# yhlleo/DWC-GAN

Hardware: AMD Instinct MI355X
Metric: CelebA 128x128 training images/sec (higher is better)
Workload: dtype f32; 1 GPU; BASELINE configs[1]: CelebA-shaped 128x128, per-GPU batch 16, fp32, full iteration (dis_update + gen_update + EMA + LR step), vgg_w=0, stride-1 3x3 / 5x5 and stride-2 4x4 layers (forward, data and weight gradient) as fp32-accurate TWO-plane f16 split products on the f16 MFMA (hi + lo 2^-11 per operand, per-tensor power-of-two scales, 3 products per multiply-add, matrix-core partial sums flushed to; image_size=128, per_gpu_batch=16, global_batch=16, parallelism=dp1

## Files before the change

dwc-gan_amd/csrc/conv_fold.h:

```cpp
#pragma once
#include "conv_geom.h"

namespace {

__device__ __forceinline__ int reflect_src(int p, int n, int pad, int (&out)[3]) {
    int c = 0;
    out[c++] = p + pad;
    if (p >= 1 && p <= pad) out[c++] = pad - p;
    if (p >= n - 1 - pad && p <= n - 2) out[c++] = pad + 2 * (n - 1) - p;
    return c;
}

template <typename T>
__global__ void fold_reflect_kernel(const T* __restrict__ gp, T* __restrict__ dx, int B, int H, int W, int C4, int pad,
                                    int Wp) {
    const size_t idx = (size_t)blockIdx.x * blockDim.x + threadIdx.x;
    const size_t total = (size_t)B * H * W * C4;
    if (idx >= total) return;
    const int c = idx % C4;
    size_t r = idx / C4;
    const int w = r % W;
    r /= W;
    const int h = r % H;
    const int n = r / H;
// ... 126 lines not shown
            else e = off_right / 4 + ((size_t)(n * H + rh - pad) * pad + rw - pad - W) * C4;
            for (int p = 0; p < parts; ++p) s += ld4(ring + p * part_stride, e + c);
        }
    st4(dx, o, s);
}

template <typename T>
int fold_ring(T* dx, const float* ring, const SameDgrad& f, int B, int H, int W, int C, int pad, hipStream_t st) {
    const size_t total = (size_t)B * 2 * pad * (W + H) * (C / 4);
    hipLaunchKernelGGL(fold_ring_kernel<T>, dim3((unsigned)((total + 255) / 256)), dim3(256), 0, st, dx, ring, f.ring_elems[0],
                       f.ring_elems[0] + f.ring_elems[1], f.ring_elems[0] + f.ring_elems[1] + f.ring_elems[2], f.parts, f.ring_total,
                       B, H, W, C / 4, pad);
    DWC_LAUNCH_CHECK();
    return DWC_OK;
}

template <typename T>
__global__ __launch_bounds__(256) void splitk_reduce_kernel(const float* __restrict__ part, T* __restrict__ dst,
                                                            const float* __restrict__ bias, size_t total4, size_t stride4, int splits,
                                                            int N, int act) {
    const int nq = N >> 2;
    for (size_t i = (size_t)blockIdx.x * blockDim.x + threadIdx.x; i < total4; i += (size_t)gridDim.x * blockDim.x) {
        f32x4 s = ld4(part, i);
        for (int z = 1; z < splits; ++z) s += ld4(part, (size_t)z * stride4 + i);
        const int c4 = i % nq;
        if (bias) s += ld4(bias, c4);
#pragma unroll
        for (int k = 0; k < 4; ++k) s[k] = dwc_act_apply(s[k], act, c4 * 4 + k);
        st4(dst, i, s);
    }
}

template <typename T>
int splitk_reduce(const float* part, T* dst, const float* bias, size_t dst_elems, int splits, int N, int act, hipStream_t st) {
    const size_t total4 = dst_elems / 4;
    size_t blocks = (total4 + 255) / 256;
    if (blocks > 2048) blocks = 2048;
    hipLaunchKernelGGL(splitk_reduce_kernel<T>, dim3((unsigned)blocks), dim3(256), 0, st, part, dst, bias, total4, total4, splits, N, act);
    DWC_LAUNCH_CHECK();
    return DWC_OK;
}

template <typename T>
__global__ void weight_prepare_fwd_kernel(const float* __restrict__ w, T* __restrict__ out, int Cout, int Cin, int KHW,
                                          int cout_pad, int cin_pad, int Kp) {
    const size_t idx = (size_t)blockIdx.x * blockDim.x + threadIdx.x;
    if (idx >= (size_t)cout_pad * Kp) return;
    const int k = idx % Kp, co = idx / Kp;
    const int ci = k % cin_pad, tap = k / cin_pad;
    float v = 0.f;
    if (co < Cout && ci < Cin && tap < KHW) v = w[((size_t)co * Cin + ci) * KHW + tap];
    out[idx] = (T)v;
}

template <typename T>
__global__ void weight_prepare_dgrad_kernel(const float* __restrict__ w, T* __restrict__ out, int Cout, int Cin, int KH, int KW,
                                            int stride, int cout_pad, int cin_pad, int Kp) {
    const size_t idx = (size_t)blockIdx.x * blockDim.x + threadIdx.x;
    const size_t per_class = (size_t)cin_pad * Kp;
    const int classes = stride == 1 ? 1 : 4;
    if (idx >= per_class * classes) return;
// ... 49 lines not shown
```

dwc-gan_amd/csrc/conv_geom.h:

```cpp
#pragma once
#include <stdio.h>
#include <stdlib.h>
#include <string.h>

#include "dwc_common.h"

namespace {

struct Gather {
    const void* src;
    int SH, SW, SC, logSC;
    int OH, OW;
    int logOW, logOHW;
    int KH, KW, kw_magic;
    int mul_h, mul_w, kstep, off_h, off_w;
    int reflect;
    int M, K;
    int tap_t;
};

struct Scatter {
    void* dst;
    int N;
    int OHf, OWf, os;
// ... 10 lines not shown
    Gather g;
    Scatter o;
    const void* w;
    int kt0, kt1, tiles, tiles_n;
    int oph, opw;
};
struct StripSet {
    Strip s[8];
    int kt_per_part;
    size_t part_stride;
};

__global__ void wgrad_reduce_kernel(const float* __restrict__ slab, float* __restrict__ dw, int splits, int K, int N, int Cin,
                                    int KHW, int cin_real, int cout_real) {
    const size_t idx = (size_t)blockIdx.x * blockDim.x + threadIdx.x;
    if (idx >= (size_t)K * N) return;
    const int co = idx % N;
    const int k = idx / N;
    const int ci = k % Cin, tap = k / Cin;
    if (co >= cout_real || ci >= cin_real) return;
    float s = 0.f;
    for (int z = 0; z < splits; ++z) s += slab[(size_t)z * K * N + idx];
    dw[((size_t)co * cin_real + ci) * KHW + tap] = s;
}

__global__ __launch_bounds__(256) void wgrad_reduce_wide_kernel(const float* __restrict__ slab, float* __restrict__ dw, int splits, int K, int N,
                                                                int Cin, int KHW, int cin_real, int cout_real) {
    __shared__ float part[8][32];
    const int e = threadIdx.x & 31, g = threadIdx.x >> 5;
    const size_t total = (size_t)K * N;
    const size_t idx = (size_t)blockIdx.x * 32 + e;
    const int per = (splits + 7) / 8;
    const int z0 = g * per, z1 = min(splits, z0 + per);
    float s = 0.f;
    if (idx < total) {
        const float* p = slab + idx;
        int z = z0;
        for (; z + 8 <= z1; z += 8) {
            float v[8];
#pragma unroll
            for (int u = 0; u < 8; ++u) v[u] = p[(size_t)(z + u) * total];
#pragma unroll
            for (int u = 0; u < 8; ++u) s += v[u];
        }
        for (; z < z1; ++z) s += p[(size_t)z * total];
    }
// ... 3 lines not shown
#pragma unroll
    for (int q = 1; q < 8; ++q) s += part[q][e];
    const int co = idx % N;
    const int k = idx / N;
    const int ci = k % Cin, tap = k / Cin;
    if (co >= cout_real || ci >= cin_real) return;
    dw[((size_t)co * cin_real + ci) * KHW + tap] = s;
}

inline bool wgrad_reduce_takes_wide(int splits, int K, int N) { return splits >= 16 && (size_t)K * N <= 262144; }

inline bool wgrad_reduce_wide(const float* slab, float* dw, int splits, int K, int N, int Cin, int KHW, int cin_real, int cout_real,
                              hipStream_t st) {
    const size_t total = (size_t)K * N;
    if (!wgrad_reduce_takes_wide(splits, K, N)) return false;
    hipLaunchKernelGGL(wgrad_reduce_wide_kernel, dim3((unsigned)((total + 31) / 32)), dim3(256), 0, st, slab, dw, splits, K, N, Cin, KHW,
                       cin_real, cout_real);
    return true;
}

inline void wgrad_reduce(const float* slab, float* dw, int splits, int K, int N, int Cin, int KHW, int cin_real, int cout_real,
                         hipStream_t st) {
    if (wgrad_reduce_wide(slab, dw, splits, K, N, Cin, KHW, cin_real, cout_real, st)) return;
    const size_t total = (size_t)K * N;
    hipLaunchKernelGGL(wgrad_reduce_kernel, dim3((unsigned)((total + 255) / 256)), dim3(256), 0, st, slab, dw, splits, K, N, Cin, KHW,
                       cin_real, cout_real);
}

int kw_magic_for(int KW, int max_tap) {
    const int magic = (65536 + KW - 1) / KW;
    for (int tp = 0; tp <= max_tap; ++tp)
        if (((tp * magic) >> 16) != tp / KW) return -1;
    return magic;
}

constexpr int NUM_CU = 256;
struct Plan {
    int bm, bn, splits, kt_per_split;
};

struct TileCand { int bm, bn, resident; float f; };

template <size_t NC>
Plan plan_gemm(int M, int N, int K, int classes, int bk, const TileCand (&cands)[NC], int split_below) {
    const int nk = (K + bk - 1) / bk;
    Plan best = {128, 32, 1, nk};
    float best_cost = 3.0e38f;
    auto valid = [N](const TileCand& c) {
        if (N <= 32) return c.bn == 32;
// ... 312 lines not shown
```

dwc-gan_amd/csrc/conv_halo_bf16.hip:

```cpp
#include <type_traits>

#include "conv_geom.h"

namespace {

typedef __bf16 bf16;
typedef __bf16 bf16x8 __attribute__((ext_vector_type(8)));
typedef __bf16 bf16x4 __attribute__((ext_vector_type(4)));

constexpr int BK = 64;
constexpr int TB = 16;

__device__ __forceinline__ bf16x4 pack4h(float a, float b, float c, float d) {
    bf16x4 r;
    r[0] = (bf16)a; r[1] = (bf16)b; r[2] = (bf16)c; r[3] = (bf16)d;
    return r;
}

struct HaloArgs {
    const bf16* x;
    const bf16* w;
    const float* bias;
    const bf16* add;
    bf16* y;
// ... 460 lines not shown
    hipStream_t st = (hipStream_t)stream;
    const dim3 grid((Cin / (bn == 128 ? 64 : 128)) * a.n_tiles * a.tap_groups * splits);
#ifdef DWC_DEV_ABLATIONS
    static const int dbg = getenv("DWC_WGRAD_HALO_DBG") ? atoi(getenv("DWC_WGRAD_HALO_DBG")) : 0;
    if (K == 3 && dbg == 4) hipLaunchKernelGGL((wgrad_halo_kernel<3, 128, 4>), grid, dim3(512), 0, st, a);
    else
#endif
    const char* he = getenv("DWC_WGRAD_HALF");
    const int half = he ? atoi(he) : 1;
    if (zero) {
        if (K == 3) hipLaunchKernelGGL((wgrad_halo_kernel<3, 128, 0, 0, -1, 0, 0, true>), grid, dim3(512), 0, st, a);
        else if (K == 4) hipLaunchKernelGGL((wgrad_halo_kernel<4, 128, 0, 0, -1, 0, 0, true>), grid, dim3(512), 0, st, a);
        else if (bn == 128 && half) hipLaunchKernelGGL((wgrad_halo_kernel<5, 128, 0, 0, -1, 0, 1, true>), grid, dim3(512), 0, st, a);
        else if (bn == 128) hipLaunchKernelGGL((wgrad_halo_kernel<5, 128, 0, 0, -1, 0, 0, true>), grid, dim3(512), 0, st, a);
        else if (half) hipLaunchKernelGGL((wgrad_halo_kernel<5, 64, 0, 0, -1, 0, 1, true>), grid, dim3(512), 0, st, a);
        else hipLaunchKernelGGL((wgrad_halo_kernel<5, 64, 0, 0, -1, 0, 0, true>), grid, dim3(512), 0, st, a);
    } else if (K == 3) hipLaunchKernelGGL((wgrad_halo_kernel<3, 128>), grid, dim3(512), 0, st, a);
    else if (K == 4) hipLaunchKernelGGL((wgrad_halo_kernel<4, 128>), grid, dim3(512), 0, st, a);
    else if (bn == 128 && half) hipLaunchKernelGGL((wgrad_halo_kernel<5, 128, 0, 0, -1, 0, 1>), grid, dim3(512), 0, st, a);
    else if (bn == 128) hipLaunchKernelGGL((wgrad_halo_kernel<5, 128>), grid, dim3(512), 0, st, a);
    else if (half) hipLaunchKernelGGL((wgrad_halo_kernel<5, 64, 0, 0, -1, 0, 1>), grid, dim3(512), 0, st, a);
    else hipLaunchKernelGGL((wgrad_halo_kernel<5, 64>), grid, dim3(512), 0, st, a);
    DWC_LAUNCH_CHECK();
    const size_t total = (size_t)K * K * Cin * Cout;
    hipLaunchKernelGGL(wgrad_reduce_kernel, dim3((total + 255) / 256), dim3(256), 0, st, (const float*)ws, dw_oihw, splits,
                       K * K * Cin, Cout, Cin, K * K, cin_real, cout_real);
    DWC_LAUNCH_CHECK();
    return DWC_OK;
}

int dwc_bf16_conv2d_wgrad_halo(const void* x, const void* dy, float* dw_oihw, int B, int H, int W, int Cin, int Cout, int K,
                               int cin_real, int cout_real, void* ws, size_t ws_bytes, void* stream) {
    return wgrad_halo_run(x, dy, dw_oihw, B, H, W, Cin, Cout, K, cin_real, cout_real, ws, ws_bytes, stream, false);
}

int dwc_bf16_conv2d_wgrad_halo_zeropad(const void* x, const void* dy, float* dw_oihw, int B, int H, int W, int Cin, int Cout, int K,
                                       int cin_real, int cout_real, void* ws, size_t ws_bytes, void* stream) {
    if (!x || !dy || !dw_oihw) return DWC_EINVAL;
    return wgrad_halo_run(x, dy, dw_oihw, B, H, W, Cin, Cout, K, cin_real, cout_real, ws, ws_bytes, stream, true);
}

}
```

dwc-gan_amd/csrc/conv_halo_x3.hip:

```cpp
#include <type_traits>

#include "conv_geom.h"

namespace {

typedef __bf16 bf16;
typedef __bf16 bf16x8 __attribute__((ext_vector_type(8)));
typedef unsigned int u32x2 __attribute__((ext_vector_type(2)));

constexpr int TB = 16;
constexpr int CS = 16;

typedef float f32x2 __attribute__((ext_vector_type(2)));
__device__ __forceinline__ void split3(f32x4 v, u32x2& p0, u32x2& p1, u32x2& p2) {
#pragma unroll
    for (int k = 0; k < 2; ++k) {
        const f32x2 x = {v[2 * k], v[2 * k + 1]};
        const f32x2 hb = {__uint_as_float(__float_as_uint(x[0]) & 0xffff0000u), __uint_as_float(__float_as_uint(x[1]) & 0xffff0000u)};
        const f32x2 r = x - hb;
        const f32x2 mb = {__uint_as_float(__float_as_uint(r[0]) & 0xffff0000u), __uint_as_float(__float_as_uint(r[1]) & 0xffff0000u)};
        const f32x2 l = r - mb;
        p0[k] = __builtin_amdgcn_perm(__float_as_uint(x[1]), __float_as_uint(x[0]), 0x07060302u);
        p1[k] = __builtin_amdgcn_perm(__float_as_uint(r[1]), __float_as_uint(r[0]), 0x07060302u);
        p2[k] = __builtin_amdgcn_perm(__float_as_uint(l[1]), __float_as_uint(l[0]), 0x07060302u);
// ... 988 lines not shown
            }
            asm volatile("s_waitcnt lgkmcnt(0)" ::: "memory");
            __builtin_amdgcn_s_barrier();
            buf ^= 1;
            cur = nxt;
            nxt = unit_next(nxt);
        }
    }
    const int Ktot = KS * KS * a.Cin;
    float* out = a.slab + (size_t)(split * HALVES + half_id) * Ktot * a.N;
#pragma unroll
    for (int kh = 0; kh < KS; ++kh) {
        const int tap = kh * KS + kw;
#pragma unroll
        for (int r = 0; r < 16; ++r) {
            const int k = tap * a.Cin + cs * CIW + ci_tile * 32 + (r & 3) + 8 * (r >> 2) + 4 * hi;
            if constexpr (NPL == 2) out[(size_t)k * a.N + tn * BN + co_tile * 32 + l31] = acc[kh][r] * sx.inv * sdy.inv;
            else out[(size_t)k * a.N + tn * BN + co_tile * 32 + l31] = acc[kh][r] + lo[kh][r];
        }
    }
#endif
}

__global__ void x3_wgrad_reduce_kernel(const float* __restrict__ slab, float* __restrict__ dw, int splits, int K, int N, int Cin, int KHW,
                                       int cin_real, int cout_real) {
    const size_t idx = (size_t)blockIdx.x * blockDim.x + threadIdx.x;
    if (idx >= (size_t)K * N) return;
    const int co = idx % N;
    const int k = idx / N;
    const int ci = k % Cin, tap = k / Cin;
    if (co >= cout_real || ci >= cin_real) return;
    const float* p = slab + idx;
    const size_t stride = (size_t)K * N;
    float s = 0.f;
    int z = 0;
    for (; z + 4 <= splits; z += 4) {
        const float v0 = p[(size_t)z * stride], v1 = p[(size_t)(z + 1) * stride], v2 = p[(size_t)(z + 2) * stride],
                    v3 = p[(size_t)(z + 3) * stride];
        s += v0;
        s += v1;
        s += v2;
        s += v3;
    }
    for (; z < splits; ++z) s += p[(size_t)z * stride];
    dw[((size_t)co * cin_real + ci) * KHW + tap] = s;
}

static int x3_wgrad_ciw() { return 64; }

int x3_wgrad_bn(int B, int H, int W, int Cin, int Cout, int K) {
    if (K == 4) {
        if (B <= 0 || H < 8 || W < 32 || (H % 8) || (W % 32) || Cin < 64 || (Cin % 64)) return 0;
    } else if (B <= 0 || (K != 3 && K != 5) || H < 8 || W < 16 || (H % 8) || (W % 16) || Cin < 64 || (Cin % 64)) return 0;
    if ((size_t)B * H * W * Cin * 4 >= 0xffffffffull || (size_t)B * H * W * Cout * 4 >= 0xffffffffull) return 0;
    if (Cout >= 128 && !(Cout % 128)) return 128;
    return (Cout >= 64 && !(Cout % 64)) ? 64 : 0;
}

void x3_wgrad_plan(int B, int H, int W, int Cin, int Cout, int K, int bn, int npl, int* splits, int* ups) {
    const int ciw = x3_wgrad_ciw();
    const int roles = (Cin / ciw) * (Cout / bn) * K;
    const int units = K == 4 ? B * (H / 8) * (W / 32) : B * (H / 8) * (W / 16);
    const int cus = (npl == 2 && K != 5 && (long)units * roles >= 8L * 512) ? 512 : 256;
    const int smax = units / 4 > 0 ? units / 4 : 1;
    int s = 1;
    double best = 0.0;
    for (int c = 1; c <= smax && c * roles <= 2 * cus; ++c) {
        const int wgs = c * roles, rounds = (wgs + cus - 1) / cus;
        const double fill = (double)wgs / (rounds * cus) / (rounds > 1 ? 1.05 : 1.0);
// ... 337 lines not shown
    X3WgradArgs a;
    a.x = x; a.dy = dy; a.slab = (float*)ws;
    a.xs = (const unsigned long long*)xs; a.xs_epoch = xs_epoch; a.dys = (const unsigned long long*)dys; a.dys_epoch = dys_epoch;
    a.B = B; a.H = H; a.W = W; a.Cin = Cin; a.N = Cout;
    if (K == 4) {
        a.units_x = W / 32; a.units_per_img = (H / 8) * (W / 32);
    } else {
        a.units_x = W / 16; a.units_per_img = (H / 8) * (W / 16);
    }
    a.total_units = B * a.units_per_img; a.units_per_split = ups;
    a.n_tiles = Cout / bn;
    const int ciw = x3_wgrad_ciw();
    a.roles = (Cin / ciw) * a.n_tiles * K;
    hipStream_t st = (hipStream_t)stream;
    const dim3 grid(a.roles * splits);
    if (K == 4) {
        if (bn == 128) hipLaunchKernelGGL((wgrad_x3_kernel<4, 128, 64, 2, NPL, ZP>), grid, dim3(512), 0, st, a);
        else hipLaunchKernelGGL((wgrad_x3_kernel<4, 64, 64, 2, NPL, ZP>), grid, dim3(512), 0, st, a);
    } else if (K == 3 && bn == 128) hipLaunchKernelGGL((wgrad_x3_kernel<3, 128, 64, 2, NPL, ZP>), grid, dim3(512), 0, st, a);
    else if (K == 3) hipLaunchKernelGGL((wgrad_x3_kernel<3, 64, 64, 2, NPL, ZP>), grid, dim3(512), 0, st, a);
    else if (bn == 128) hipLaunchKernelGGL((wgrad_x3_kernel<5, 128, 64, 2, NPL, ZP>), grid, dim3(512), 0, st, a);
    else hipLaunchKernelGGL((wgrad_x3_kernel<5, 64, 64, 2, NPL, ZP>), grid, dim3(512), 0, st, a);
    DWC_LAUNCH_CHECK();
    const size_t total = (size_t)K * K * Cin * Cout;
    hipLaunchKernelGGL(x3_wgrad_reduce_kernel, dim3((total + 255) / 256), dim3(256), 0, st, (const float*)ws, dw_oihw, splits * halves,
                       K * K * Cin, Cout, Cin, K * K, cin_real, cout_real);
    DWC_LAUNCH_CHECK();
    return DWC_OK;
}

extern "C" {

int dwc_x3_conv2d_wgrad(const float* x, const float* dy, float* dw_oihw, int B, int H, int W, int Cin, int Cout, int K, int cin_real,
                        int cout_real, void* ws, size_t ws_bytes, void* stream) {
    return x3_wgrad_impl<3>(x, nullptr, 0, dy, nullptr, 0, dw_oihw, B, H, W, Cin, Cout, K, cin_real, cout_real, ws, ws_bytes, stream);
}
int dwc_h2_conv2d_wgrad(const float* x, const void* x_amax, unsigned x_epoch, const float* dy, const void* dy_amax, unsigned dy_epoch,
                        float* dw_oihw, int B, int H, int W, int Cin, int Cout, int K, int cin_real, int cout_real, void* ws, size_t ws_bytes,
                        void* stream) {
    return x3_wgrad_impl<2>(x, x_amax, x_epoch, dy, dy_amax, dy_epoch, dw_oihw, B, H, W, Cin, Cout, K, cin_real, cout_real, ws, ws_bytes, stream);
}
int dwc_x3_conv2d_wgrad_zeropad(const float* x, const float* dy, float* dw_oihw, int B, int H, int W, int Cin, int Cout, int K,
                                int cin_real, int cout_real, void* ws, size_t ws_bytes, void* stream) {
    return x3_wgrad_impl<3, true>(x, nullptr, 0, dy, nullptr, 0, dw_oihw, B, H, W, Cin, Cout, K, cin_real, cout_real, ws, ws_bytes, stream);
}
int dwc_h2_conv2d_wgrad_zeropad(const float* x, const void* x_amax, unsigned x_epoch, const float* dy, const void* dy_amax,
                                unsigned dy_epoch, float* dw_oihw, int B, int H, int W, int Cin, int Cout, int K, int cin_real,
                                int cout_real, void* ws, size_t ws_bytes, void* stream) {
    return x3_wgrad_impl<2, true>(x, x_amax, x_epoch, dy, dy_amax, dy_epoch, dw_oihw, B, H, W, Cin, Cout, K, cin_real, cout_real, ws, ws_bytes,
// ... 5 lines not shown
```

dwc-gan_amd/csrc/conv_igemm.hip:

```cpp
#include <type_traits>

#include <atomic>

#include "conv_im2col_entry.h"

namespace {

constexpr int BK = 32;


__device__ __attribute__((aligned(16))) float g_zero_page[64];

#ifdef DWC_CLOCK_PROBE
__device__ unsigned long long g_clock_probe[2];
struct ClockProbe {
    long long c0, r0;
    __device__ ClockProbe() : c0(clock64()), r0(wall_clock64()) {}
    __device__ ~ClockProbe() {
        if (blockIdx.x == 0 && blockIdx.y == 0 && blockIdx.z == 0 && threadIdx.x == 0) {
            atomicAdd(&g_clock_probe[0], (unsigned long long)(clock64() - c0));
            atomicAdd(&g_clock_probe[1], (unsigned long long)(wall_clock64() - r0));
        }
    }
};
// ... 618 lines not shown
    static int fold_image(const float* dxp, float* dx, int B, int H, int W, int C, int pad, hipStream_t st) {
        return fold_reflect(dxp, dx, B, H, W, C / 4, pad, W + 2 * pad, st);
    }

    static bool band_args_bad(const void* dxp, const void* dx, int , int , int C) { return !dxp || !dx || C <= 0; }
};

}

#define DWC_F32_NAME(x) dwc_##x
DWC_IM2COL_EXPORTS(DWC_F32_NAME, Im2colF32, float)
#undef DWC_F32_NAME

extern "C" {

int dwc_version(void) { return DWC_ABI_VERSION; }

int dwc_x3_gemm_mode(int mode) {
    const int prev = x3_mode();
    if (mode >= 0) g_x3_mode.store(mode & 3, std::memory_order_relaxed);
    return prev;
}

int dwc_reflect_pad_adjoint_pitch(const float* dxp, float* dx, int B, int H, int W, int C, int pad, int pitch, void* stream) {
    if (B <= 0 || H <= 0 || W <= 0 || C <= 0 || (C & 3) || pad < 0 || pad >= H || pad >= W || pitch < W + 2 * pad) return DWC_EINVAL;
    return fold_reflect(dxp, dx, B, H, W, C / 4, pad, pitch, (hipStream_t)stream);
}

}

#ifdef DWC_CLOCK_PROBE
extern "C" int dwc_debug_clock_probe(unsigned long long* out, int reset) {
    if (hipMemcpyFromSymbol(out, HIP_SYMBOL(g_clock_probe), 16) != hipSuccess) return DWC_ELAUNCH;
    if (reset) {
        const unsigned long long z[2] = {0, 0};
        if (hipMemcpyToSymbol(HIP_SYMBOL(g_clock_probe), z, 16) != hipSuccess) return DWC_ELAUNCH;
    }
    return 0;
}
#endif
```

dwc-gan_amd/csrc/dwc_common.h:

```cpp
#pragma once
#include <hip/hip_runtime.h>
#include <stdint.h>
#include "../../include/dwcgan_hip.h"

typedef float f32x16 __attribute__((ext_vector_type(16)));
typedef float f32x4 __attribute__((ext_vector_type(4)));
typedef __bf16 dwc_bf16;
typedef __bf16 dwc_bf16x4 __attribute__((ext_vector_type(4)));
typedef __bf16 dwc_bf16x8 __attribute__((ext_vector_type(8)));

#ifdef __HIPCC__
__device__ __forceinline__ f32x4 ld4(const float* p, size_t i4) { return reinterpret_cast<const f32x4*>(p)[i4]; }
__device__ __forceinline__ f32x4 ld4(const dwc_bf16* p, size_t i4) {
    const dwc_bf16x4 v = reinterpret_cast<const dwc_bf16x4*>(p)[i4];
    return f32x4{(float)v[0], (float)v[1], (float)v[2], (float)v[3]};
}
__device__ __forceinline__ void st4(float* p, size_t i4, f32x4 v) { reinterpret_cast<f32x4*>(p)[i4] = v; }
__device__ __forceinline__ void st4(dwc_bf16* p, size_t i4, f32x4 v) {
    dwc_bf16x4 r;
    r[0] = (dwc_bf16)v[0]; r[1] = (dwc_bf16)v[1]; r[2] = (dwc_bf16)v[2]; r[3] = (dwc_bf16)v[3];
    reinterpret_cast<dwc_bf16x4*>(p)[i4] = r;
}
#endif

#ifdef __HIPCC__
// ... 72 lines not shown
}
struct H2Scale { float s, inv; };
__device__ __forceinline__ H2Scale h2_scale(const unsigned long long* slot, unsigned epoch) {
    const unsigned long long v = *slot;
    unsigned e = ((unsigned)v >> 23) & 0xffu;
    H2Scale r;
    if (e == 0xffu) {
        r.s = r.inv = 1.f;
    } else {
        e = min(max(e, 27u), 254u);
        r.s = __uint_as_float((267u - e) << 23);
        r.inv = __uint_as_float((e - 13u) << 23);
    }
    if ((unsigned)(v >> 32) != epoch) r.s = r.inv = __builtin_nanf("");
    return r;
}
#endif

#define DWC_LAUNCH_CHECK()                                   \
    do {                                                     \
        if (hipGetLastError() != hipSuccess) return DWC_ELAUNCH; \
    } while (0)

static inline int dwc_ilog2_exact(int v) {
    if (v <= 0 || (v & (v - 1))) return -1;
    int l = 0;
    while ((1 << l) < v) ++l;
    return l;
}

__device__ __forceinline__ float dwc_wave_sum(float v) {
#pragma unroll
    for (int off = 32; off > 0; off >>= 1) v += __shfl_xor(v, off, 64);
    return v;
}

__device__ __forceinline__ float dwc_block_sum_256(float v, float* sm) {
    v = dwc_wave_sum(v);
    const int wave = threadIdx.x >> 6;
    __syncthreads();
    if ((threadIdx.x & 63) == 0) sm[wave] = v;
    __syncthreads();
    return sm[0] + sm[1] + sm[2] + sm[3];
}

__device__ __forceinline__ float dwc_act_apply(float v, int act, int ch) {
// ... 29 lines not shown
```

dwc-gan_amd/csrc/weight_refresh.hip:

```cpp
#include "dwc_common.h"

namespace {

typedef __bf16 bf16;

__device__ __forceinline__ float im2col_elem(const dwc_refresh_desc& d, size_t idx, bool dgrad) {
    const float* w = d.src;
    if (!dgrad) {
        const int KHW = d.KH * d.KW;
        const int k = idx % d.Kp, co = idx / d.Kp;
        const int ci = k % d.cin_pad, tap = k / d.cin_pad;
        return (co < d.Cout && ci < d.Cin && tap < KHW) ? w[((size_t)co * d.Cin + ci) * KHW + tap] : 0.f;
    }
    const size_t per_class = (size_t)d.cin_pad * d.Kp;
    const int cls = idx / per_class;
    const size_t r = idx % per_class;
    const int k = r % d.Kp, ci = r / d.Kp;
    const int co = k % d.cout_pad, tapo = k / d.cout_pad;
    int kh, kw;
    bool ok = co < d.Cout && ci < d.Cin;
    if (d.stride == 1) {
        ok = ok && tapo < d.KH * d.KW;
        kh = d.KH - 1 - tapo / d.KW;
        kw = d.KW - 1 - tapo % d.KW;
// ... 81 lines not shown
                const int kc = cs * CS + j;
                float v = 0.f;
                if (d.kind == DWC_REFRESH_X3_FWD) {
                    if (row < d.Cout && kc < d.Cin) v = d.src[(((size_t)row * d.Cin + kc) * K + kh) * K + kw];
                } else {
                    if (row < d.Cin && kc < d.Cout) v = d.src[(((size_t)kc * d.Cin + row) * K + (K - 1 - kh)) * K + (K - 1 - kw)];
                }
                const unsigned hb = __float_as_uint(v) & 0xffff0000u;
                const float r1 = v - __uint_as_float(hb);
                const unsigned mb = __float_as_uint(r1) & 0xffff0000u;
                const float r2 = r1 - __uint_as_float(mb);
                unsigned short* o = reinterpret_cast<unsigned short*>(d.dst);
                const size_t base = ((size_t)(tap * ncs + cs) * 3 * rows + row) * CS + (j ^ (((row >> 3) & 1) << 3));
                o[base] = (unsigned short)(hb >> 16);
                o[base + (size_t)rows * CS] = (unsigned short)(mb >> 16);
                o[base + 2 * (size_t)rows * CS] = (unsigned short)(__float_as_uint(r2) >> 16);
                break;
            }
            default: break;
        }
    }
}

}

extern "C" {

int dwc_weight_refresh_multi(const dwc_refresh_desc* descs_dev, const int* chunk_desc_dev, const unsigned* chunk_start_dev, int n_chunks,
                             int has_h2, unsigned epoch, void* stream) {
    if (n_chunks <= 0) return DWC_OK;
    if (!descs_dev || !chunk_desc_dev || !chunk_start_dev) return DWC_EINVAL;
    if (has_h2) {
        hipLaunchKernelGGL(weight_refresh_multi_kernel<true>, dim3(n_chunks), dim3(256), 0, (hipStream_t)stream, descs_dev, chunk_desc_dev,
                           chunk_start_dev, epoch);
        DWC_LAUNCH_CHECK();
    }
    hipLaunchKernelGGL(weight_refresh_multi_kernel<false>, dim3(n_chunks), dim3(256), 0, (hipStream_t)stream, descs_dev, chunk_desc_dev,
                       chunk_start_dev, epoch);
    DWC_LAUNCH_CHECK();
    return DWC_OK;
}

}
```

dwc-gan_amd/hipdwc/_lib.py:

```python
import ctypes
import os

_HERE = os.path.dirname(os.path.abspath(__file__))
LIB_PATH = os.environ.get("DWC_HIP_LIB") or os.path.join(os.path.dirname(_HERE), "lib", "libdwcgan_hip.so")

c_fp = ctypes.c_void_p
c_int = ctypes.c_int
c_sz = ctypes.c_size_t
c_f = ctypes.c_float
c_u = ctypes.c_uint


class AdvSpec(ctypes.Structure):
    _fields_ = [("target", c_f * 4), ("w_src", c_f * 4), ("w_cls", c_f * 4)]


BN_MAX_SEGMENTS = 8


TXT_MAX_LAYERS = 4


class TxtLayers(ctypes.Structure):
    _fields_ = [("n", c_int), ("out", c_fp * TXT_MAX_LAYERS), ("c", c_fp * TXT_MAX_LAYERS)]
# ... 190 lines not shown
    "dwc_batchnorm_ws_bytes": (c_sz, [c_int] * 4),
    "dwc_batchnorm_fwd": (c_int, [c_fp] * 8 + [c_int] * 4 + [c_f, c_f, c_int, c_int, BnOrder, c_fp, c_sz, c_fp]),
    "dwc_batchnorm_bwd": (c_int, [c_fp] * 9 + [c_int] * 6 + [c_fp, c_sz, c_fp]),
    "dwc_batchnorm_fwd_amax": (c_int, [c_fp] * 8 + [c_int] * 4 + [c_f, c_f, c_int, c_int, BnOrder, c_fp, c_sz, c_fp, c_u, c_fp]),
    "dwc_batchnorm_bwd_amax": (c_int, [c_fp] * 9 + [c_int] * 6 + [c_fp, c_sz, c_fp, c_u, c_fp]),
    "dwc_bf16_batchnorm_fwd": (c_int, [c_fp] * 8 + [c_int] * 4 + [c_f, c_f, c_int, c_int, BnOrder, c_fp, c_sz, c_fp]),
    "dwc_bf16_batchnorm_bwd": (c_int, [c_fp] * 9 + [c_int] * 6 + [c_fp, c_sz, c_fp]),
    "dwc_syncbn_ws_bytes": (c_sz, [c_int] * 4),
    "dwc_syncbn_moments": (c_int, [c_fp, c_fp] + [c_int] * 4 + [c_fp, c_sz, c_fp]),
    "dwc_bf16_syncbn_moments": (c_int, [c_fp, c_fp] + [c_int] * 4 + [c_fp, c_sz, c_fp]),
    "dwc_syncbn_finalise": (c_int, [c_fp, c_int] + [c_fp] * 4 + [c_int, c_int, c_f, c_f, BnOrder, c_fp]),
    "dwc_syncbn_apply": (c_int, [c_fp] * 6 + [c_int] * 5 + [c_fp]),
    "dwc_syncbn_apply_amax": (c_int, [c_fp] * 6 + [c_int] * 5 + [c_fp, c_u, c_fp]),
    "dwc_bf16_syncbn_apply": (c_int, [c_fp] * 6 + [c_int] * 5 + [c_fp]),
    "dwc_syncbn_bwd_sums": (c_int, [c_fp] * 9 + [c_int] * 5 + [c_fp, c_sz, c_fp]),
    "dwc_bf16_syncbn_bwd_sums": (c_int, [c_fp] * 9 + [c_int] * 5 + [c_fp, c_sz, c_fp]),
    "dwc_syncbn_bwd_apply": (c_int, [c_fp] * 7 + [c_int, ctypes.c_long, c_fp] + [c_int] * 5 + [c_fp]),
    "dwc_syncbn_bwd_apply_amax": (c_int, [c_fp] * 7 + [c_int, ctypes.c_long, c_fp] + [c_int] * 5 + [c_fp, c_u, c_fp]),
    "dwc_bf16_syncbn_bwd_apply": (c_int, [c_fp] * 7 + [c_int, ctypes.c_long, c_fp] + [c_int] * 5 + [c_fp]),
    "dwc_conv2d_fwd_plan": (c_int, [c_int] * 9 + [c_fp]),
    "dwc_conv2d_bwd_weight_plan": (c_int, [c_int] * 9 + [c_fp]),
    "dwc_bf16_conv2d_fwd_plan": (c_int, [c_int] * 9 + [c_fp]),
    "dwc_bf16_conv2d_bwd_weight_plan": (c_int, [c_int] * 9 + [c_fp]),
    "dwc_conv2d_bwd_weight_zeropad_ws_bytes": (c_sz, [c_int] * 9),
    "dwc_conv2d_bwd_weight_zeropad": (c_int, [c_fp, c_fp, c_fp] + [c_int] * 11 + [c_fp, c_sz, c_fp]),
    "dwc_conv2d_bwd_data_crop_ws_bytes": (c_sz, [c_int] * 9),
    "dwc_conv2d_bwd_data_crop": (c_int, [c_fp, c_fp, c_fp] + [c_int] * 9 + [c_fp, c_sz, c_fp]),
    "dwc_bf16_conv2d_bwd_weight_zeropad_ws_bytes": (c_sz, [c_int] * 9),
    "dwc_bf16_conv2d_bwd_weight_zeropad": (c_int, [c_fp, c_fp, c_fp] + [c_int] * 11 + [c_fp, c_sz, c_fp]),
    "dwc_bf16_conv2d_bwd_data_crop_ws_bytes": (c_sz, [c_int] * 9),
    "dwc_bf16_conv2d_bwd_data_crop": (c_int, [c_fp, c_fp, c_fp] + [c_int] * 9 + [c_fp, c_sz, c_fp]),
    "dwc_x3_conv2d_wgrad_zeropad": (c_int, [c_fp, c_fp, c_fp] + [c_int] * 8 + [c_fp, c_sz, c_fp]),
    "dwc_h2_conv2d_wgrad_zeropad": (c_int, [c_fp, c_fp, c_u, c_fp, c_fp, c_u, c_fp] + [c_int] * 8 + [c_fp, c_sz, c_fp]),
    "dwc_bf16_conv2d_wgrad_halo_zeropad": (c_int, [c_fp, c_fp, c_fp] + [c_int] * 8 + [c_fp, c_sz, c_fp]),
    "dwc_x3_conv2d_s2_ws_zeropad": (c_int, [c_fp] * 4 + [c_int] * 7 + [c_fp, c_sz, c_fp, c_fp]),
    "dwc_h2_conv2d_s2_ws_zeropad": (c_int, [c_fp, c_fp, c_u, c_fp, c_fp, c_fp, c_fp, c_u] + [c_int] * 7 + [c_fp, c_sz, c_fp, c_fp]),
    "dwc_bf16_conv2d_s2_halo_zeropad": (c_int, [c_fp, c_fp, c_fp, c_fp] + [c_int] * 6 + [c_fp]),
    "dwc_txt_operand_fwd": (c_int, [c_fp] * 6 + [c_int] * 6 + [c_fp]),
    "dwc_txt_operand_bwd": (c_int, [c_fp] * 8 + [c_int] * 5 + [c_fp]),
    "dwc_txt_prev_state": (c_int, [c_fp, c_fp] + [c_int] * 3 + [c_fp]),
    "dwc_txt_inter_fwd": (c_int, [c_fp] * 4 + [c_int] * 3 + [c_fp]),
    "dwc_txt_inter_bwd": (c_int, [c_fp] * 7 + [c_int, c_fp] + [c_int] * 3 + [c_fp]),
    "dwc_txt_states_fwd": (c_int, [TxtLayers, c_fp, c_fp, c_fp] + [c_int] * 3 + [c_fp]),
    "dwc_txt_states_bwd": (c_int, [c_fp, c_fp, c_fp, TxtLayers] + [c_int] * 3 + [c_fp]),
}

# ... 48 lines not shown
```

include/dwcgan_hip.h:

```cpp
#ifndef DWCGAN_HIP_H
#define DWCGAN_HIP_H

#include <stddef.h>
#include <stdint.h>

#ifdef __cplusplus
extern "C" {
#endif

#define DWC_OK 0
#define DWC_EINVAL (-1)
#define DWC_EWORKSPACE (-2)
#define DWC_ELAUNCH (-3)

#define DWC_ACT_NONE 0
#define DWC_ACT_RELU 1
#define DWC_ACT_LRELU 2
#define DWC_ACT_TANH 3
#define DWC_ACT_SIGMOID 4
#define DWC_ACT_HEADS 5
#define DWC_ACT_HEADS8 6

#define DWC_ABI_VERSION 11
int dwc_version(void);
// ... 25 lines not shown
int dwc_conv2d_bwd_data_ring(const float* dy, const float* w_dgrad, const float* w_dgrad_t, float* dx,
                             int B, int H, int W, int Cin, int Cout, int KH, int KW, int pad,
                             void* ws, size_t ws_bytes, void* stream);
size_t dwc_conv2d_bwd_data_image_ws_bytes(int B, int H, int W, int Cout, int KH, int KW, int pad);
int dwc_conv2d_bwd_data_image(const float* dy, const float* w_wide, float* dx,
                              int B, int H, int W, int Cout, int KH, int KW, int pad,
                              void* ws, size_t ws_bytes, void* stream);
size_t dwc_conv2d_bwd_weight_ws_bytes(int B, int H, int W, int Cin, int Cout, int KH, int KW,
                                      int stride, int pad);
int dwc_conv2d_bwd_weight(const float* x, const float* dy, float* dw_oihw,
                          int B, int H, int W, int Cin, int Cout, int KH, int KW, int stride, int pad,
                          int cin_real, int cout_real, void* ws, size_t ws_bytes, void* stream);
int dwc_conv2d_fwd_ex(const float* x, const float* w_prepared, const float* bias, float* y,
                      int B, int H, int W, int Cin, int Cout, int KH, int KW,
                      int stride_h, int stride_w, int pad_h, int pad_w, int act, void* stream);
size_t dwc_conv2d_bwd_weight_ex_ws_bytes(int B, int H, int W, int Cin, int Cout, int KH, int KW,
                                         int stride_h, int stride_w, int pad_h, int pad_w);
int dwc_conv2d_bwd_weight_ex(const float* x, const float* dy, float* dw_oihw,
                             int B, int H, int W, int Cin, int Cout, int KH, int KW,
                             int stride_h, int stride_w, int pad_h, int pad_w,
                             int cin_real, int cout_real, void* ws, size_t ws_bytes, void* stream);
int dwc_conv2d_fwd_plan(int B, int H, int W, int Cin, int Cout, int KH, int KW, int stride, int pad, int out[4]);
int dwc_conv2d_bwd_weight_plan(int B, int H, int W, int Cin, int Cout, int KH, int KW, int stride, int pad, int out[4]);
size_t dwc_act_bwd_bias_ws_bytes(int rows, int C);
int dwc_act_bwd_bias(const float* dy, const float* y, float* g, float* db, int rows, int C, int act,
                     void* ws, size_t ws_bytes, void* stream);

int dwc_norm_act_ok(int act);
size_t dwc_instnorm_ws_bytes(int B, int HW, int C);
int dwc_instnorm_fwd(const float* x, const float* gamma, const float* beta, const float* residual,
                     float* y, float* mean, float* rstd, int B, int HW, int C, float eps, int relu,
                     void* ws, size_t ws_bytes, void* stream);
int dwc_instnorm_bwd(const float* dy, const float* x, const float* mean, const float* rstd,
                     const float* gamma, const float* beta, float* dx, float* dgamma, float* dbeta,
                     int B, int HW, int C, int relu, void* ws, size_t ws_bytes, void* stream);

int dwc_linear_small_ok(int M, int N, int K);
int dwc_linear_small_fwd(const float* x, const float* w, const float* bias, float* y, int M, int N, int K, int relu, void* stream);
int dwc_linear_small_bwd(const float* dy, const float* y_relu, const float* x, const float* w, float* dx, float* dw, float* db, int M,
                         int N, int K, void* stream);
int dwc_linear_small_fwd_act(const float* x, const float* w, const float* bias, float* y, int M, int N, int K, int act, float slope,
                             void* stream);
int dwc_linear_small_bwd_act(const float* dy, const float* y_act, const float* x, const float* w, float* dx, float* dw, float* db,
                             int M, int N, int K, int act, float slope, void* stream);

size_t dwc_layernorm_ws_bytes(int B, int HW, int C);
// ... 414 lines not shown
```

Before: 381.1 images/s.

## Tile weight-gradient split reduction through LDS and batch split-K loads

Adds a tiled weight-gradient slab reduction that reads coalesced along output channels, including vectorised f32x4 loads, accumulates up to 8 splits in flight, then transposes through LDS to write OIHW weights contiguously. The split-K reduce now issues four partial loads at once, and the H2 weight-refresh amax pass gets a linear vectorised kernel. All three are on by default and can be turned off with an environment variable. The aim is to cut the latency-bound, poorly coalesced reduction passes; the cost is extra LDS use, more launch-shape heuristics and a getenv call on every launch.

```diff
diff --git a/dwc-gan_amd/csrc/conv_fold.h b/dwc-gan_amd/csrc/conv_fold.h
--- a/dwc-gan_amd/csrc/conv_fold.h
+++ b/dwc-gan_amd/csrc/conv_fold.h
@@ -172,6 +172,31 @@
     const int nq = N >> 2;
     for (size_t i = (size_t)blockIdx.x * blockDim.x + threadIdx.x; i < total4; i += (size_t)gridDim.x * blockDim.x) {
         f32x4 s = ld4(part, i);
+        int z = 1;
+        for (; z + 4 <= splits; z += 4) {
+            const f32x4 v0 = ld4(part, (size_t)z * stride4 + i), v1 = ld4(part, (size_t)(z + 1) * stride4 + i),
+                        v2 = ld4(part, (size_t)(z + 2) * stride4 + i), v3 = ld4(part, (size_t)(z + 3) * stride4 + i);
+            s += v0;
+            s += v1;
+            s += v2;
+            s += v3;
+        }
+        for (; z < splits; ++z) s += ld4(part, (size_t)z * stride4 + i);
+        const int c4 = i % nq;
+        if (bias) s += ld4(bias, c4);
+#pragma unroll
+        for (int k = 0; k < 4; ++k) s[k] = dwc_act_apply(s[k], act, c4 * 4 + k);
+        st4(dst, i, s);
+    }
+}
+
+template <typename T>
+__global__ __launch_bounds__(256) void splitk_reduce_chained_kernel(const float* __restrict__ part, T* __restrict__ dst,
+                                                                    const float* __restrict__ bias, size_t total4, size_t stride4,
+                                                                    int splits, int N, int act) {
+    const int nq = N >> 2;
+    for (size_t i = (size_t)blockIdx.x * blockDim.x + threadIdx.x; i < total4; i += (size_t)gridDim.x * blockDim.x) {
+        f32x4 s = ld4(part, i);
         for (int z = 1; z < splits; ++z) s += ld4(part, (size_t)z * stride4 + i);
         const int c4 = i % nq;
         if (bias) s += ld4(bias, c4);
@@ -186,7 +211,11 @@
     const size_t total4 = dst_elems / 4;
     size_t blocks = (total4 + 255) / 256;
     if (blocks > 2048) blocks = 2048;
-    hipLaunchKernelGGL(splitk_reduce_kernel<T>, dim3((unsigned)blocks), dim3(256), 0, st, part, dst, bias, total4, total4, splits, N, act);
+    if (dwc_weight_passes_on())
+        hipLaunchKernelGGL(splitk_reduce_kernel<T>, dim3((unsigned)blocks), dim3(256), 0, st, part, dst, bias, total4, total4, splits, N, act);
+    else
+        hipLaunchKernelGGL(splitk_reduce_chained_kernel<T>, dim3((unsigned)blocks), dim3(256), 0, st, part, dst, bias, total4, total4, splits,
+                           N, act);
     DWC_LAUNCH_CHECK();
     return DWC_OK;
 }
diff --git a/dwc-gan_amd/csrc/conv_geom.h b/dwc-gan_amd/csrc/conv_geom.h
--- a/dwc-gan_amd/csrc/conv_geom.h
+++ b/dwc-gan_amd/csrc/conv_geom.h
@@ -56,6 +56,111 @@
     float s = 0.f;
     for (int z = 0; z < splits; ++z) s += slab[(size_t)z * K * N + idx];
     dw[((size_t)co * cin_real + ci) * KHW + tap] = s;
+}
+
+__global__ void x3_wgrad_reduce_kernel(const float* __restrict__ slab, float* __restrict__ dw, int splits, int K, int N, int Cin, int KHW,
+                                       int cin_real, int cout_real) {
+    const size_t idx = (size_t)blockIdx.x * blockDim.x + threadIdx.x;
+    if (idx >= (size_t)K * N) return;
+    const int co = idx % N;
+    const int k = idx / N;
+    const int ci = k % Cin, tap = k / Cin;
+    if (co >= cout_real || ci >= cin_real) return;
+    const float* p = slab + idx;
+    const size_t stride = (size_t)K * N;
+    float s = 0.f;
+    int z = 0;
+    for (; z + 4 <= splits; z += 4) {
+        const float v0 = p[(size_t)z * stride], v1 = p[(size_t)(z + 1) * stride], v2 = p[(size_t)(z + 2) * stride],
+                    v3 = p[(size_t)(z + 3) * stride];
+        s += v0;
+        s += v1;
+        s += v2;
+        s += v3;
+    }
+    for (; z < splits; ++z) s += p[(size_t)z * stride];
+    dw[((size_t)co * cin_real + ci) * KHW + tap] = s;
+}
+
+constexpr int WGRAD_TILE_CO = 32;
+template <typename T>
+__global__ __launch_bounds__(1024) void wgrad_reduce_tiled_kernel(const float* __restrict__ slab, float* __restrict__ dw, int splits, int K,
+                                                                  int N, int Cin, int KHW, int cin_real, int cout_real, int ci_t) {
+    extern __shared__ float wgrad_tile[];
+    const int co0 = blockIdx.x * WGRAD_TILE_CO, ci0 = blockIdx.y * ci_t;
+    const int nci = min(ci_t, cin_real - ci0);
+    const int nco = min(WGRAD_TILE_CO, cout_real - co0);
+    const int pitch = ci_t * KHW + 1;
+    const int rows = nci * KHW;
+    constexpr int V = sizeof(T) / sizeof(float), QN = WGRAD_TILE_CO / V;
+    const int q = threadIdx.x % QN;
+    const size_t stride = (size_t)K * N;
+    if (V * q < nco) {
+        for (int r = threadIdx.x / QN; r < rows; r += blockDim.x / QN) {
+            const int tap = r / nci, cil = r - tap * nci;
+            const float* p = slab + (size_t)(tap * Cin + ci0 + cil) * N + co0 + V * q;
+            T s = (T)(0.f);
+            for (int z = 0; z < splits; z += 8) {
+                const int n = min(8, splits - z);
+                T v[8];
+#pragma unroll
+                for (int u = 0; u < 8; ++u) v[u] = *reinterpret_cast<const T*>(p + (size_t)(z + min(u, n - 1)) * stride);
+#pragma unroll
+                for (int u = 0; u < 8; ++u)
+                    if (u < n) s += v[u];
+            }
+            float* t = wgrad_tile + (V * q) * pitch + cil * KHW + tap;
+            if constexpr (V == 1) {
+                t[0] = s;
+            } else {
+#pragma unroll
+                for (int j = 0; j < V; ++j) t[j * pitch] = s[j];
+            }
+        }
+    }
+    __syncthreads();
+    for (int e = threadIdx.x; e < nco * rows; e += blockDim.x) {
+        const int c = e / rows, o = e - c * rows;
+        dw[((size_t)(co0 + c) * cin_real + ci0) * KHW + o] = wgrad_tile[c * pitch + o];
+    }
+}
+
+inline bool wgrad_reduce_tiled_scalar(int K, int N) { return (size_t)K * N <= 262144; }
+
+inline int wgrad_reduce_ci_tile(int KHW, int cin_real, int cout_real, bool scalar) {
+    if (KHW > 160) return 0;
+    int t = 64;
+    while (t > 1 && t * KHW > 160) t >>= 1;
+    const int tiles_co = (cout_real + WGRAD_TILE_CO - 1) / WGRAD_TILE_CO;
+    while (t > 4 && tiles_co * ((cin_real + t - 1) / t) < 256) t >>= 1;
+    while (scalar && t > 1 && (t * KHW > 32 || tiles_co * ((cin_real + t - 1) / t) < 2 * 256)) t >>= 1;
+    return t;
+}
+
+inline void wgrad_reduce_plain(const float* slab, float* dw, int splits, int K, int N, int Cin, int KHW, int cin_real, int cout_real,
+                               bool four_in_flight, hipStream_t st) {
+    const bool scalar = wgrad_reduce_tiled_scalar(K, N);
+    const int ci_t = wgrad_reduce_ci_tile(KHW, cin_real, cout_real, scalar);
+    if (dwc_weight_passes_on() && ci_t > 0 && !(N & 3) && !((uintptr_t)slab & 15) && cin_real > 0 && cout_real > 0 && K == KHW * Cin) {
+        const dim3 grid((cout_real + WGRAD_TILE_CO - 1) / WGRAD_TILE_CO, (cin_real + ci_t - 1) / ci_t);
+        int threads = (min(ci_t, cin_real) * KHW * (scalar ? 32 : 8) + 63) / 64 * 64;
+        if (threads > 1024) threads = 1024;
+        const size_t lds = WGRAD_TILE_CO * (ci_t * KHW + 1) * sizeof(float);
+        if (scalar)
+            hipLaunchKernelGGL(wgrad_reduce_tiled_kernel<float>, grid, dim3(threads), lds, st, slab, dw, splits, K, N, Cin, KHW, cin_real,
+                               cout_real, ci_t);
+        else
+            hipLaunchKernelGGL(wgrad_reduce_tiled_kernel<f32x4>, grid, dim3(threads), lds, st, slab, dw, splits, K, N, Cin, KHW, cin_real,
+                               cout_real, ci_t);
+        return;
+    }
+    const size_t total = (size_t)K * N;
+    if (four_in_flight)
+        hipLaunchKernelGGL(x3_wgrad_reduce_kernel, dim3((unsigned)((total + 255) / 256)), dim3(256), 0, st, slab, dw, splits, K, N, Cin, KHW,
+                           cin_real, cout_real);
+    else
+        hipLaunchKernelGGL(wgrad_reduce_kernel, dim3((unsigned)((total + 255) / 256)), dim3(256), 0, st, slab, dw, splits, K, N, Cin, KHW,
+                           cin_real, cout_real);
 }
 
 __global__ __launch_bounds__(256) void wgrad_reduce_wide_kernel(const float* __restrict__ slab, float* __restrict__ dw, int splits, int K, int N,
@@ -105,9 +210,7 @@
 inline void wgrad_reduce(const float* slab, float* dw, int splits, int K, int N, int Cin, int KHW, int cin_real, int cout_real,
                          hipStream_t st) {
     if (wgrad_reduce_wide(slab, dw, splits, K, N, Cin, KHW, cin_real, cout_real, st)) return;
-    const size_t total = (size_t)K * N;
-    hipLaunchKernelGGL(wgrad_reduce_kernel, dim3((unsigned)((total + 255) / 256)), dim3(256), 0, st, slab, dw, splits, K, N, Cin, KHW,
-                       cin_real, cout_real);
+    wgrad_reduce_plain(slab, dw, splits, K, N, Cin, KHW, cin_real, cout_real, false, st);
 }
 
 int kw_magic_for(int KW, int max_tap) {
diff --git a/dwc-gan_amd/csrc/conv_halo_bf16.hip b/dwc-gan_amd/csrc/conv_halo_bf16.hip
--- a/dwc-gan_amd/csrc/conv_halo_bf16.hip
+++ b/dwc-gan_amd/csrc/conv_halo_bf16.hip
@@ -506,9 +506,7 @@
     else if (half) hipLaunchKernelGGL((wgrad_halo_kernel<5, 64, 0, 0, -1, 0, 1>), grid, dim3(512), 0, st, a);
     else hipLaunchKernelGGL((wgrad_halo_kernel<5, 64>), grid, dim3(512), 0, st, a);
     DWC_LAUNCH_CHECK();
-    const size_t total = (size_t)K * K * Cin * Cout;
-    hipLaunchKernelGGL(wgrad_reduce_kernel, dim3((total + 255) / 256), dim3(256), 0, st, (const float*)ws, dw_oihw, splits,
-                       K * K * Cin, Cout, Cin, K * K, cin_real, cout_real);
+    wgrad_reduce_plain((const float*)ws, dw_oihw, splits, K * K * Cin, Cout, Cin, K * K, cin_real, cout_real, false, st);
     DWC_LAUNCH_CHECK();
     return DWC_OK;
 }
diff --git a/dwc-gan_amd/csrc/conv_halo_x3.hip b/dwc-gan_amd/csrc/conv_halo_x3.hip
--- a/dwc-gan_amd/csrc/conv_halo_x3.hip
+++ b/dwc-gan_amd/csrc/conv_halo_x3.hip
@@ -1034,29 +1034,6 @@
 #endif
 }
 
-__global__ void x3_wgrad_reduce_kernel(const float* __restrict__ slab, float* __restrict__ dw, int splits, int K, int N, int Cin, int KHW,
-                                       int cin_real, int cout_real) {
-    const size_t idx = (size_t)blockIdx.x * blockDim.x + threadIdx.x;
-    if (idx >= (size_t)K * N) return;
-    const int co = idx % N;
-    const int k = idx / N;
-    const int ci = k % Cin, tap = k / Cin;
-    if (co >= cout_real || ci >= cin_real) return;
-    const float* p = slab + idx;
-    const size_t stride = (size_t)K * N;
-    float s = 0.f;
-    int z = 0;
-    for (; z + 4 <= splits; z += 4) {
-        const float v0 = p[(size_t)z * stride], v1 = p[(size_t)(z + 1) * stride], v2 = p[(size_t)(z + 2) * stride],
-                    v3 = p[(size_t)(z + 3) * stride];
-        s += v0;
-        s += v1;
-        s += v2;
-        s += v3;
-    }
-    for (; z < splits; ++z) s += p[(size_t)z * stride];
-    dw[((size_t)co * cin_real + ci) * KHW + tap] = s;
-}
 
 static int x3_wgrad_ciw() { return 64; }
 
@@ -1440,9 +1417,7 @@
     else if (bn == 128) hipLaunchKernelGGL((wgrad_x3_kernel<5, 128, 64, 2, NPL, ZP>), grid, dim3(512), 0, st, a);
     else hipLaunchKernelGGL((wgrad_x3_kernel<5, 64, 64, 2, NPL, ZP>), grid, dim3(512), 0, st, a);
     DWC_LAUNCH_CHECK();
-    const size_t total = (size_t)K * K * Cin * Cout;
-    hipLaunchKernelGGL(x3_wgrad_reduce_kernel, dim3((total + 255) / 256), dim3(256), 0, st, (const float*)ws, dw_oihw, splits * halves,
-                       K * K * Cin, Cout, Cin, K * K, cin_real, cout_real);
+    wgrad_reduce_plain((const float*)ws, dw_oihw, splits * halves, K * K * Cin, Cout, Cin, K * K, cin_real, cout_real, true, st);
     DWC_LAUNCH_CHECK();
     return DWC_OK;
 }
diff --git a/dwc-gan_amd/csrc/conv_igemm.hip b/dwc-gan_amd/csrc/conv_igemm.hip
--- a/dwc-gan_amd/csrc/conv_igemm.hip
+++ b/dwc-gan_amd/csrc/conv_igemm.hip
@@ -664,6 +664,26 @@
     return prev;
 }
 
+int dwc_wgrad_slab_reduce(const float* slab, float* dw, int splits, int KHW, int Cin, int N, int cin_real, int cout_real, int route,
+                          void* stream) {
+    if (!slab || !dw || splits <= 0 || KHW <= 0 || Cin <= 0 || N <= 0 || (N & 3) || cin_real <= 0 || cin_real > Cin || cout_real <= 0 ||
+        cout_real > N || route < 0 || route > 2)
+        return DWC_EINVAL;
+    hipStream_t st = (hipStream_t)stream;
+    if (route == 0) wgrad_reduce(slab, dw, splits, KHW * Cin, N, Cin, KHW, cin_real, cout_real, st);
+    else wgrad_reduce_plain(slab, dw, splits, KHW * Cin, N, Cin, KHW, cin_real, cout_real, route == 2, st);
+    DWC_LAUNCH_CHECK();
+    return DWC_OK;
+}
+
+int dwc_splitk_reduce(const float* part, void* dst, const float* bias, size_t dst_elems, int splits, int N, int act, int dst_bf16,
+                      void* stream) {
+    if (!part || !dst || !dst_elems || (dst_elems & 3) || splits <= 0 || N <= 0 || (N & 3) || act < DWC_ACT_NONE || act > DWC_ACT_HEADS8)
+        return DWC_EINVAL;
+    if (dst_bf16) return splitk_reduce(part, (dwc_bf16*)dst, bias, dst_elems, splits, N, act, (hipStream_t)stream);
+    return splitk_reduce(part, (float*)dst, bias, dst_elems, splits, N, act, (hipStream_t)stream);
+}
+
 int dwc_reflect_pad_adjoint_pitch(const float* dxp, float* dx, int B, int H, int W, int C, int pad, int pitch, void* stream) {
     if (B <= 0 || H <= 0 || W <= 0 || C <= 0 || (C & 3) || pad < 0 || pad >= H || pad >= W || pitch < W + 2 * pad) return DWC_EINVAL;
     return fold_reflect(dxp, dx, B, H, W, C / 4, pad, pitch, (hipStream_t)stream);
diff --git a/dwc-gan_amd/csrc/dwc_common.h b/dwc-gan_amd/csrc/dwc_common.h
--- a/dwc-gan_amd/csrc/dwc_common.h
+++ b/dwc-gan_amd/csrc/dwc_common.h
@@ -1,6 +1,7 @@
 #pragma once
 #include <hip/hip_runtime.h>
 #include <stdint.h>
+#include <stdlib.h>
 #include "../../include/dwcgan_hip.h"
 
 typedef float f32x16 __attribute__((ext_vector_type(16)));
@@ -119,6 +120,11 @@
         if (hipGetLastError() != hipSuccess) return DWC_ELAUNCH; \
     } while (0)
 
+static inline bool dwc_weight_passes_on() {
+    const char* e = getenv("DWC_WEIGHT_PASSES");
+    return !(e && atoi(e) == 0);
+}
+
 static inline int dwc_ilog2_exact(int v) {
     if (v <= 0 || (v & (v - 1))) return -1;
     int l = 0;
diff --git a/dwc-gan_amd/csrc/weight_refresh.hip b/dwc-gan_amd/csrc/weight_refresh.hip
--- a/dwc-gan_amd/csrc/weight_refresh.hip
+++ b/dwc-gan_amd/csrc/weight_refresh.hip
@@ -127,6 +127,30 @@
     }
 }
 
+__global__ __launch_bounds__(256) void weight_refresh_amax_linear_kernel(const dwc_refresh_desc* __restrict__ descs,
+                                                                         const int* __restrict__ chunk_desc,
+                                                                         const unsigned* __restrict__ chunk_start, unsigned epoch) {
+    const dwc_refresh_desc d = descs[chunk_desc[blockIdx.x]];
+    if (d.kind != DWC_REFRESH_H2_FWD && d.kind != DWC_REFRESH_H2_DGRAD) return;
+    const size_t src_n = (size_t)d.Cout * d.Cin * d.KH * d.KH;
+    const size_t i0 = chunk_start[blockIdx.x];
+    const size_t i1 = min(src_n, i0 + DWC_OPT_CHUNK);
+    if (i0 >= i1) return;
+    unsigned long long* h2_slot =
+        reinterpret_cast<unsigned long long*>(reinterpret_cast<float*>(reinterpret_cast<unsigned short*>(d.dst) + 2 * d.n_items) + 2);
+    unsigned am = 0;
+    size_t s0 = i0;
+    if (!(reinterpret_cast<uintptr_t>(d.src + i0) & 15)) {
+        s0 = i0 + ((i1 - i0) & ~(size_t)3);
+        for (size_t idx = i0 + 4 * threadIdx.x; idx < s0; idx += 4 * 256) {
+            const f32x4 v = *reinterpret_cast<const f32x4*>(d.src + idx);
+            am = max(max(am, dwc_abs_bits(v[0])), max(dwc_abs_bits(v[1]), max(dwc_abs_bits(v[2]), dwc_abs_bits(v[3]))));
+        }
+    }
+    for (size_t idx = s0 + threadIdx.x; idx < i1; idx += 256) am = max(am, dwc_abs_bits(d.src[idx]));
+    dwc_amax_wave_publish(h2_slot, epoch, am);
+}
+
 }
 
 extern "C" {
@@ -136,8 +160,12 @@
     if (n_chunks <= 0) return DWC_OK;
     if (!descs_dev || !chunk_desc_dev || !chunk_start_dev) return DWC_EINVAL;
     if (has_h2) {
-        hipLaunchKernelGGL(weight_refresh_multi_kernel<true>, dim3(n_chunks), dim3(256), 0, (hipStream_t)stream, descs_dev, chunk_desc_dev,
-                           chunk_start_dev, epoch);
+        if (dwc_weight_passes_on())
+            hipLaunchKernelGGL(weight_refresh_amax_linear_kernel, dim3(n_chunks), dim3(256), 0, (hipStream_t)stream, descs_dev, chunk_desc_dev,
+                               chunk_start_dev, epoch);
+        else
+            hipLaunchKernelGGL(weight_refresh_multi_kernel<true>, dim3(n_chunks), dim3(256), 0, (hipStream_t)stream, descs_dev, chunk_desc_dev,
+                               chunk_start_dev, epoch);
         DWC_LAUNCH_CHECK();
     }
     hipLaunchKernelGGL(weight_refresh_multi_kernel<false>, dim3(n_chunks), dim3(256), 0, (hipStream_t)stream, descs_dev, chunk_desc_dev,
diff --git a/dwc-gan_amd/hipdwc/_lib.py b/dwc-gan_amd/hipdwc/_lib.py
--- a/dwc-gan_amd/hipdwc/_lib.py
+++ b/dwc-gan_amd/hipdwc/_lib.py
@@ -236,6 +236,8 @@
     "dwc_conv2d_bwd_weight_plan": (c_int, [c_int] * 9 + [c_fp]),
     "dwc_bf16_conv2d_fwd_plan": (c_int, [c_int] * 9 + [c_fp]),
     "dwc_bf16_conv2d_bwd_weight_plan": (c_int, [c_int] * 9 + [c_fp]),
+    "dwc_wgrad_slab_reduce": (c_int, [c_fp, c_fp] + [c_int] * 7 + [c_fp]),
+    "dwc_splitk_reduce": (c_int, [c_fp, c_fp, c_fp, c_sz] + [c_int] * 4 + [c_fp]),
     "dwc_conv2d_bwd_weight_zeropad_ws_bytes": (c_sz, [c_int] * 9),
     "dwc_conv2d_bwd_weight_zeropad": (c_int, [c_fp, c_fp, c_fp] + [c_int] * 11 + [c_fp, c_sz, c_fp]),
     "dwc_conv2d_bwd_data_crop_ws_bytes": (c_sz, [c_int] * 9),
diff --git a/include/dwcgan_hip.h b/include/dwcgan_hip.h
--- a/include/dwcgan_hip.h
+++ b/include/dwcgan_hip.h
@@ -71,6 +71,10 @@
                              int cin_real, int cout_real, void* ws, size_t ws_bytes, void* stream);
 int dwc_conv2d_fwd_plan(int B, int H, int W, int Cin, int Cout, int KH, int KW, int stride, int pad, int out[4]);
 int dwc_conv2d_bwd_weight_plan(int B, int H, int W, int Cin, int Cout, int KH, int KW, int stride, int pad, int out[4]);
+int dwc_wgrad_slab_reduce(const float* slab, float* dw, int splits, int KHW, int Cin, int N, int cin_real, int cout_real, int route,
+                          void* stream);
+int dwc_splitk_reduce(const float* part, void* dst, const float* bias, size_t dst_elems, int splits, int N, int act, int dst_bf16,
+                      void* stream);
 size_t dwc_act_bwd_bias_ws_bytes(int rows, int C);
 int dwc_act_bwd_bias(const float* dy, const float* y, float* g, float* db, int rows, int C, int act,
                      void* ws, size_t ws_bytes, void* stream);
```

Measured after the change: 383.9 images/s, median of 6. About the same (+0.7%).
